# adri-romsor/iterative_inference_segm

Hardware: AMD Instinct MI355X
Metric: refined images/s (FCN-8 + standard DAE, 10-step iterative inference, 224x224, 11 classes) (higher is better)
Workload: dtype f32; 1 GPU; BASELINE configs[1]: FCN-8 + standard DAE (f64c1p2, pool4, trackind, skip), 224x224x3, batch 64/GPU, 10 steps, step 0.1, early stop off; per batch: pred_fcn_fn, val_fn, pred_dae_fn+val_fn, refine, val_fn; global_batch=64, parallelism=dp1

## Files before the change

include/iiseg.h:

```cpp
#ifndef IISEG_H
#define IISEG_H

#include <stdint.h>

#ifdef __cplusplus
extern "C" {
#endif

typedef enum iiseg_status {
    IISEG_OK = 0,
    IISEG_ERR_NULL = -1,
    IISEG_ERR_SHAPE = -2,
    IISEG_ERR_ALIGN = -3,
    IISEG_ERR_LAUNCH = -4,
    IISEG_ERR_UNSUPPORTED = -5
} iiseg_status;

const char* iiseg_strerror(int status);
const char* iiseg_last_hip_error(void);
int iiseg_abi_version(void);
const char* iiseg_target_arch(void);

int iiseg_profile_begin(int capacity);
int iiseg_profile_count(void);
// ... 14 lines not shown
    uint32_t flags;
    int32_t Kpad, Mpad;
    int32_t out_ctot, out_c0;
    int32_t out_H, out_W, out_y0, out_x0;
    int32_t tile_y0, tile_x0;
} iiseg_conv_desc;

int iiseg_conv_ktab_entries(const iiseg_conv_desc* d);
int iiseg_conv_plan(iiseg_conv_desc* d);

int iiseg_conv_pack_f32(void* stream, const iiseg_conv_desc* d, const float* w,
                        int64_t stride_o, int64_t stride_c, float* wp, int32_t* ktab);

int iiseg_conv_f32(void* stream, const iiseg_conv_desc* d, const float* x1, const float* x2,
                   const float* pre, const float* pooled, const float* wp, const int32_t* ktab,
                   const float* bias, const float* add, float* out);

int iiseg_conv_small_supported(const iiseg_conv_desc* d);
int iiseg_conv_pool_supported(const iiseg_conv_desc* d);
int iiseg_conv_pool_f32(void* stream, const iiseg_conv_desc* d, const float* x1, const float* x2,
                        const float* pre, const float* pooled, const float* wp, const int32_t* ktab,
                        const float* bias, const float* add, float* out, float* pool_out);

int iiseg_conv_mask_supported(const iiseg_conv_desc* d);
int iiseg_conv_mask_f32(void* stream, const iiseg_conv_desc* d, const float* x1, const float* x2,
                        const float* pre, const float* pooled, const uint8_t* mask_in,
                        const float* wp, const int32_t* ktab, const float* bias, const float* add,
                        float* out, float* pool_out, uint8_t* mask_out);

int iiseg_conv_halo_seam(int on);
int64_t iiseg_conv_halo_seam_launches(void);

int iiseg_conv_bnrelu_supported(const iiseg_conv_desc* d);
int iiseg_conv_bnrelu_f32(void* stream, const iiseg_conv_desc* d, const float* x, int64_t x_bstride,
                          const float* beta, const float* gamma, const float* mean,
                          const float* inv_std, const float* wp, const int32_t* ktab,
                          const float* bias, float* out);

#define IISEG_WINO_INPUT 1u
#define IISEG_WINO_GEMM 2u
#define IISEG_WINO_OUTPUT 4u
#define IISEG_WINO_ALL 7u
#define IISEG_WINO_FUSED 8u
int iiseg_conv_wino_supported(const iiseg_conv_desc* d);
int64_t iiseg_conv_wino_weight_elems(const iiseg_conv_desc* d);
int64_t iiseg_conv_wino_workspace_elems(const iiseg_conv_desc* d);
int iiseg_conv_wino_pack_f32(void* stream, const iiseg_conv_desc* d, const float* w,
                             int64_t stride_o, int64_t stride_c, float* U);
int iiseg_conv_wino_f32(void* stream, const iiseg_conv_desc* d, const float* x1, const float* x2,
                        const float* pre, const float* pooled, const float* U, const float* bias,
                        const float* add, float* workspace, float* out, uint32_t stages);
int iiseg_conv_wino_input_wide(int on);
int iiseg_conv_wino_input_path(const iiseg_conv_desc* d, int mask_bytes);
int iiseg_conv_wino_pool_supported(const iiseg_conv_desc* d);
int iiseg_conv_wino_mask_f32(void* stream, const iiseg_conv_desc* d, const float* x1, const float* x2,
                             const float* pre, const float* pooled, const uint8_t* mask_in,
                             const float* U, const float* bias, const float* add, float* workspace,
                             float* out, float* pool_out, uint8_t* mask_out, uint32_t stages);

int iiseg_conv_wino_bf16_supported(const iiseg_conv_desc* d);
int64_t iiseg_conv_wino_bf16_weight_bytes(const iiseg_conv_desc* d);
int64_t iiseg_conv_wino_bf16_workspace_bytes(const iiseg_conv_desc* d);
int iiseg_conv_wino_bf16_pack(void* stream, const iiseg_conv_desc* d, const float* w,
                              int64_t stride_o, int64_t stride_c, void* U16);
int iiseg_conv_wino_bf16(void* stream, const iiseg_conv_desc* d, const float* x1, const float* x2,
                         const float* pre, const float* pooled, const void* U16, const float* bias,
                         const float* add, void* workspace, float* out, uint32_t stages);

int iiseg_conv_gemm_bf16_supported(const iiseg_conv_desc* d);
int64_t iiseg_conv_gemm_bf16_weight_bytes(const iiseg_conv_desc* d);
int64_t iiseg_conv_gemm_bf16_workspace_bytes(const iiseg_conv_desc* d);
int iiseg_conv_gemm_bf16_pack(void* stream, const iiseg_conv_desc* d, const float* w,
                              int64_t stride_o, int64_t stride_c, void* U16);
int iiseg_conv_gemm_bf16(void* stream, const iiseg_conv_desc* d, const float* x, const void* U16,
                         const float* bias, void* workspace, float* out);

int iiseg_conv_halo_bf16_supported(const iiseg_conv_desc* d);
int64_t iiseg_conv_halo_bf16_weight_bytes(const iiseg_conv_desc* d);
int iiseg_conv_halo_bf16_pack(void* stream, const iiseg_conv_desc* d, const float* w,
                              int64_t stride_o, int64_t stride_c, void* wp16);
int iiseg_conv_halo_bf16(void* stream, const iiseg_conv_desc* d, const float* x1, const float* x2,
                         const float* pre, const float* pooled, const void* wp16, const float* bias,
                         const float* add, float* out, float* pool_out, const uint8_t* mask_in,
                         uint8_t* mask_out);

int iiseg_conv_wino_f64_supported(const iiseg_conv_desc* d);
int64_t iiseg_conv_wino_f64_weight_elems(const iiseg_conv_desc* d);
int64_t iiseg_conv_wino_f64_workspace_elems(const iiseg_conv_desc* d);
int iiseg_conv_wino_pack_f64(void* stream, const iiseg_conv_desc* d, const double* w,
                             int64_t stride_o, int64_t stride_c, double* U);
int iiseg_conv_wino_f64(void* stream, const iiseg_conv_desc* d, const double* x1, const double* x2,
                        const double* pre, const double* pooled, const double* U, const double* bias,
                        const double* add, double* workspace, double* out);

int iiseg_conv_c8_supported(const iiseg_conv_desc* d);
int iiseg_conv_c8_is_flat(const iiseg_conv_desc* d);
int iiseg_conv_c8_tiling(const iiseg_conv_desc* d, int pool, int32_t* out4);
int iiseg_conv_c8_force_tiling(int kind, int th, int tw);
int iiseg_conv_c8(void* stream, const iiseg_conv_desc* d, const void* x1, const void* x2,
                  const uint8_t* mask_in, const void* wp16, const float* bias, const void* add,
                  int add_kind, void* out, int out_kind, void* pool_out, uint8_t* mask_out);
int iiseg_conv_c8_slice(void* stream, const iiseg_conv_desc* d, const void* x1, int32_t x1_ctot,
                        const void* x2, const uint8_t* mask_in, const void* wp16, const float* bias,
                        const void* add, int add_kind, void* out, int out_kind, void* pool_out,
                        uint8_t* mask_out);
int iiseg_unpool_c8(void* stream, const void* up, const uint8_t* mask, void* out, int BC8, int H, int W,
// ... 281 lines not shown
```

iterative_inference_segm_amd/_lib.py:

```python
import ctypes as C
import os

HERE = os.path.dirname(os.path.abspath(__file__))
LIB_PATH = os.path.join(HERE, 'libiiseg_hip.so')

ABI_VERSION = 34

CONV_RELU = 1
CONV_UNPOOL = 2
CONV_X3 = 8
CONV_TRANSPOSED2 = 4
CONV_ZINS = 16


class ConvDesc(C.Structure):
    _fields_ = [(n, C.c_int32) for n in
                ('B', 'C1', 'C2', 'H', 'W', 'Cout', 'KH', 'KW', 'pad', 'dil',
                 'oy0', 'ox0', 'OH', 'OW', 'AH', 'AW', 'ay0', 'ax0')] + \
               [('flags', C.c_uint32), ('Kpad', C.c_int32), ('Mpad', C.c_int32),
                ('out_ctot', C.c_int32), ('out_c0', C.c_int32),
                ('out_H', C.c_int32), ('out_W', C.c_int32), ('out_y0', C.c_int32),
                ('out_x0', C.c_int32), ('tile_y0', C.c_int32), ('tile_x0', C.c_int32)]


# ... 10 lines not shown
class CrfDesc(C.Structure):
    _fields_ = [(n, C.c_int32) for n in ('B', 'C', 'H', 'W', 'R')] + [('flags', C.c_uint32)] + \
               [(n, C.c_double) for n in ('sxy_g', 'w_g', 'sxy_b', 'srgb', 'w_b', 'clip')]


LOSS_CROSSENTROPY = 1
LOSS_SQUARED_ERROR = 2
OPT_RMSPROP = 0
OPT_ADAM = 1


class WgradDesc(C.Structure):
    _fields_ = [(n, C.c_int32) for n in ('B', 'Cin', 'Cout', 'H', 'W', 'K', 'dil', 'gz_H', 'gz_W', 'gz_y0',
                                         'gz_x0', 'reserved')] + [('so', C.c_int64), ('sc', C.c_int64)]


class DgradDesc(C.Structure):
    _fields_ = [(n, C.c_int32) for n in ('B', 'Cin', 'Cout', 'K', 'dil', 'OH', 'OW', 'out_H', 'out_W', 'out_y0',
                                         'out_x0', 'wy0', 'wx0', 'WH', 'WW', 'ci0', 'nci', 'gx_C', 'gx_H', 'gx_W',
                                         'gx_c0', 'gx_y0', 'gx_x0', 'reserved')] + [('so', C.c_int64), ('sc', C.c_int64)]


_vp, _i32, _i64, _f32, _f64 = C.c_void_p, C.c_int32, C.c_int64, C.c_float, C.c_double

SIGNATURES = {
    'iiseg_strerror': (C.c_char_p, [C.c_int]),
    'iiseg_last_hip_error': (C.c_char_p, []),
    'iiseg_abi_version': (C.c_int, []),
    'iiseg_profile_begin': (C.c_int, [C.c_int]),
    'iiseg_profile_count': (C.c_int, []),
    'iiseg_profile_end': (C.c_int, [C.POINTER(C.c_float), C.c_int]),
    'iiseg_target_arch': (C.c_char_p, []),
    'iiseg_conv_ktab_entries': (C.c_int, [C.POINTER(ConvDesc)]),
    'iiseg_conv_plan': (C.c_int, [C.POINTER(ConvDesc)]),
    'iiseg_conv_pack_f32': (C.c_int, [_vp, C.POINTER(ConvDesc), _vp, _i64, _i64, _vp, _vp]),
    'iiseg_conv_f32': (C.c_int, [_vp, C.POINTER(ConvDesc)] + [_vp] * 9),
    'iiseg_conv_small_supported': (C.c_int, [C.POINTER(ConvDesc)]),
    'iiseg_conv_pool_supported': (C.c_int, [C.POINTER(ConvDesc)]),
    'iiseg_conv_pool_f32': (C.c_int, [_vp, C.POINTER(ConvDesc)] + [_vp] * 10),
    'iiseg_conv_halo_seam': (C.c_int, [C.c_int]),
    'iiseg_conv_halo_seam_launches': (_i64, []),
    'iiseg_conv_mask_supported': (C.c_int, [C.POINTER(ConvDesc)]),
    'iiseg_conv_mask_f32': (C.c_int, [_vp, C.POINTER(ConvDesc)] + [_vp] * 12),
    'iiseg_conv_bnrelu_supported': (C.c_int, [C.POINTER(ConvDesc)]),
    'iiseg_conv_bnrelu_f32': (C.c_int, [_vp, C.POINTER(ConvDesc), _vp, _i64] + [_vp] * 8),
    'iiseg_conv_wino_supported': (C.c_int, [C.POINTER(ConvDesc)]),
    'iiseg_conv_wino_weight_elems': (_i64, [C.POINTER(ConvDesc)]),
    'iiseg_conv_wino_workspace_elems': (_i64, [C.POINTER(ConvDesc)]),
    'iiseg_conv_wino_pack_f32': (C.c_int, [_vp, C.POINTER(ConvDesc), _vp, _i64, _i64, _vp]),
    'iiseg_conv_wino_f32': (C.c_int, [_vp, C.POINTER(ConvDesc)] + [_vp] * 9 + [C.c_uint32]),
    'iiseg_conv_wino_pool_supported': (C.c_int, [C.POINTER(ConvDesc)]),
    'iiseg_conv_wino_input_wide': (C.c_int, [C.c_int]),
    'iiseg_conv_wino_input_path': (C.c_int, [C.POINTER(ConvDesc), C.c_int]),
    'iiseg_conv_wino_mask_f32': (C.c_int, [_vp, C.POINTER(ConvDesc)] + [_vp] * 12 + [C.c_uint32]),
    'iiseg_conv_wino_bf16_supported': (C.c_int, [C.POINTER(ConvDesc)]),
    'iiseg_conv_wino_bf16_weight_bytes': (_i64, [C.POINTER(ConvDesc)]),
    'iiseg_conv_wino_bf16_workspace_bytes': (_i64, [C.POINTER(ConvDesc)]),
    'iiseg_conv_wino_bf16_pack': (C.c_int, [_vp, C.POINTER(ConvDesc), _vp, _i64, _i64, _vp]),
    'iiseg_conv_wino_bf16': (C.c_int, [_vp, C.POINTER(ConvDesc)] + [_vp] * 9 + [C.c_uint32]),
    'iiseg_conv_gemm_bf16_supported': (C.c_int, [C.POINTER(ConvDesc)]),
    'iiseg_conv_gemm_bf16_weight_bytes': (_i64, [C.POINTER(ConvDesc)]),
    'iiseg_conv_gemm_bf16_workspace_bytes': (_i64, [C.POINTER(ConvDesc)]),
    'iiseg_conv_gemm_bf16_pack': (C.c_int, [_vp, C.POINTER(ConvDesc), _vp, _i64, _i64, _vp]),
    'iiseg_conv_gemm_bf16': (C.c_int, [_vp, C.POINTER(ConvDesc)] + [_vp] * 5),
    'iiseg_conv_halo_bf16_supported': (C.c_int, [C.POINTER(ConvDesc)]),
    'iiseg_conv_halo_bf16_weight_bytes': (_i64, [C.POINTER(ConvDesc)]),
    'iiseg_conv_halo_bf16_pack': (C.c_int, [_vp, C.POINTER(ConvDesc), _vp, _i64, _i64, _vp]),
    'iiseg_conv_halo_bf16': (C.c_int, [_vp, C.POINTER(ConvDesc)] + [_vp] * 11),
    'iiseg_conv_wino_f64_supported': (C.c_int, [C.POINTER(ConvDesc)]),
    'iiseg_conv_wino_f64_weight_elems': (_i64, [C.POINTER(ConvDesc)]),
    'iiseg_conv_wino_f64_workspace_elems': (_i64, [C.POINTER(ConvDesc)]),
    'iiseg_conv_wino_pack_f64': (C.c_int, [_vp, C.POINTER(ConvDesc), _vp, _i64, _i64, _vp]),
    'iiseg_conv_wino_f64': (C.c_int, [_vp, C.POINTER(ConvDesc)] + [_vp] * 9),
    'iiseg_conv_c8_supported': (C.c_int, [C.POINTER(ConvDesc)]),
    'iiseg_conv_c8_is_flat': (C.c_int, [C.POINTER(ConvDesc)]),
    'iiseg_conv_c8_force_tiling': (C.c_int, [C.c_int, C.c_int, C.c_int]),
    'iiseg_conv_c8_tiling': (C.c_int, [C.POINTER(ConvDesc), C.c_int, C.POINTER(C.c_int32)]),
    'iiseg_conv_c8': (C.c_int, [_vp, C.POINTER(ConvDesc)] + [_vp] * 6 + [_i32, _vp, _i32, _vp, _vp]),
    'iiseg_conv_c8_slice': (C.c_int, [_vp, C.POINTER(ConvDesc), _vp, _i32] + [_vp] * 5 + [_i32, _vp, _i32, _vp, _vp]),
    'iiseg_unpool_c8': (C.c_int, [_vp] * 4 + [C.c_int] * 7),
    'iiseg_conv_c8_m16_supported': (C.c_int, [C.POINTER(ConvDesc)]),
    'iiseg_conv_c8_m16': (C.c_int, [_vp, C.POINTER(ConvDesc), _vp, _i32] + [_vp] * 6 + [_i32]),
    'iiseg_conv_c8_m16_workspace_bytes': (_i64, [C.POINTER(ConvDesc)]),
    'iiseg_conv_c8_m16_ws': (C.c_int, [_vp, C.POINTER(ConvDesc), _vp, _i32] + [_vp] * 6 + [_i32, _vp, _i64, _vp, _vp, _f64] + [_vp] * 4 + [_i32]),
    'iiseg_conv1x1_c8_weight_bytes': (_i64, [C.c_int, C.c_int]),
    'iiseg_conv1x1_c8_pack': (C.c_int, [_vp, _vp, _i64, _i64, C.c_int, C.c_int, C.c_int, _vp]),
    'iiseg_conv1x1_c8': (C.c_int, [_vp, _vp] + [C.c_int] * 5 + [_vp] * 4 + [C.c_int, C.c_int, _vp, C.c_int, C.c_int]),
    'iiseg_bn_fold_f32': (C.c_int, [_vp] * 7 + [_i32]),
    'iiseg_bn_stats_c8_workspace_elems': (C.c_int64, [_i32]),
    'iiseg_bn_stats_c8': (C.c_int, [_vp, _vp] + [_i32] * 6 + [C.c_double, _vp, _vp, _vp]),
    'iiseg_nchw_to_c8_slice': (C.c_int, [_vp, _vp, _vp] + [_i32] * 6),
    'iiseg_c8_slice_to_nchw': (C.c_int, [_vp, _vp, _vp] + [_i32] * 6),
    'iiseg_nchw_to_c8': (C.c_int, [_vp, _vp, _vp] + [_i32] * 5),
    'iiseg_c8_to_nchw': (C.c_int, [_vp, _vp, _vp] + [_i32] * 5),
    'iiseg_pool_mask_c8': (C.c_int, [_vp, _vp, _i32, _vp, _vp] + [_i32] * 11),
    'iiseg_conv_c8_split_weights': (C.c_int, [_vp, _vp, _i64, _i64, _i32, _i32, _vp]),
    'iiseg_nchw_to_c8x3': (C.c_int, [_vp, _vp, _vp] + [_i32] * 5),
    'iiseg_c8x3_to_nchw': (C.c_int, [_vp, _vp, _vp] + [_i32] * 5),
    'iiseg_pool_mask_c8x3': (C.c_int, [_vp, _vp, _vp, _vp] + [_i32] * 12),
    'iiseg_conv_gemm_supported': (C.c_int, [C.POINTER(ConvDesc)]),
    'iiseg_conv_gemm_workspace_elems': (_i64, [C.POINTER(ConvDesc)]),
    'iiseg_conv_gemm_f32': (C.c_int, [_vp, C.POINTER(ConvDesc)] + [_vp] * 5 + [C.c_uint32]),
    'iiseg_maxpool2x2_f32': (C.c_int, [_vp, _vp, _vp, _i32, _i32, _i32]),
    'iiseg_unpool_eqmask_f32': (C.c_int, [_vp, _vp, _vp, _vp, _vp, _i32, _i32, _i32]),
    'iiseg_maxpool2x2_window_f32': (C.c_int, [_vp] * 3 + [_i32] * 7),
    'iiseg_maxpool2x2_window_f64': (C.c_int, [_vp] * 3 + [_i32] * 7),
# ... 113 lines not shown
```

iterative_inference_segm_amd/csrc/conv_wino.hip:

```cpp
#include <hip/hip_runtime.h>
#include <stdint.h>
#include <stdlib.h>
#include <atomic>
#include <type_traits>
#include "iiseg.h"
#include "common.h"
#include "conv_common.h"

using namespace iiseg;

namespace {

struct WinoParams {
    const float* x1;
    const float* x2;
    const float* pre;
    const float* pooled;
    const uint8_t* mask_in;
    int h2, w2;
    const float* U;
    const float* bias;
    const float* add;
    float* V;
    float* M;
    float* out;
    int B, C1, C2, H, W;
    int Cout, pad;
    int oy0, ox0, OH, OW;
    int ty0, tx0, nty, ntx;
    int T, Tpad;
    int Kc, Mpad;
    int AH, AW, ay0, ax0;
    int relu;
    int out_ctot, out_c0, out_H, out_W, out_y0, out_x0;
    int n_ttiles, n_mtiles;
    float* pool;
    uint8_t* mask_out;
    int pool_H, pool_W;
};

__device__ __forceinline__ float pool4(float v00, float v01, float v10, float v11) {
    const float a = v00 > v01 ? v00 : v01;
    const float b = v10 > v11 ? v10 : v11;
    return a > b ? a : b;
}

__device__ __forceinline__ void pool_store(const WinoParams& p, int b, int co, int ay, int ax,
                                           float v00, float v01, float v10, float v11) {
    const float m = pool4(v00, v01, v10, v11);
    const size_t po = ((size_t)b * p.Cout + co) * p.pool_H * p.pool_W + (size_t)(ay >> 1) * p.pool_W + (ax >> 1);
    p.pool[po] = m;
    if (p.mask_out)
        p.mask_out[po] = (uint8_t)((v00 == m ? 1u : 0u) | (v01 == m ? 2u : 0u) |
                                   (v10 == m ? 4u : 0u) | (v11 == m ? 8u : 0u));
}

constexpr int RSRC_W3 = 0x00027000;

__device__ __forceinline__ __amdgpu_buffer_rsrc_t mk_rsrc(const float* base, int bytes) {
    return __builtin_amdgcn_make_buffer_rsrc((void*)base, 0, bytes, RSRC_W3);
}

__global__ void wino_weight_kernel(const float* __restrict__ w, int64_t so, int64_t sc,
                                   float* __restrict__ U, int Cin, int Cout, int Kc, int Mpad) {
    const int64_t n = (int64_t)Kc * Mpad;
    for (int64_t i = blockIdx.x * (int64_t)blockDim.x + threadIdx.x; i < n;
         i += (int64_t)gridDim.x * blockDim.x) {
        const int c = (int)(i / Mpad), co = (int)(i % Mpad);
        double g[3][3], t[4][3];
        const bool real = c < Cin && co < Cout;
#pragma unroll
        for (int a = 0; a < 3; ++a)
#pragma unroll
            for (int b = 0; b < 3; ++b) g[a][b] = real ? (double)w[co * so + c * sc + a * 3 + b] : 0.0;
#pragma unroll
        for (int b = 0; b < 3; ++b) {
            t[0][b] = g[0][b];
            t[1][b] = 0.5 * (g[0][b] + g[1][b] + g[2][b]);
            t[2][b] = 0.5 * (g[0][b] - g[1][b] + g[2][b]);
            t[3][b] = g[2][b];
        }
#pragma unroll
        for (int a = 0; a < 4; ++a) {
            const double u0 = t[a][0], u1 = 0.5 * (t[a][0] + t[a][1] + t[a][2]),
                         u2 = 0.5 * (t[a][0] - t[a][1] + t[a][2]), u3 = t[a][2];
            U[(int64_t)(a * 4 + 0) * n + i] = (float)u0;
            U[(int64_t)(a * 4 + 1) * n + i] = (float)u1;
            U[(int64_t)(a * 4 + 2) * n + i] = (float)u2;
            U[(int64_t)(a * 4 + 3) * n + i] = (float)u3;
        }
    }
}

constexpr int ICH = 4;
template <bool UNPOOL, int PY, int PX, bool MB = false>
__global__ __launch_bounds__(256) void wino_input_kernel(const WinoParams p) {
    const int t = blockIdx.x * 256 + threadIdx.x;
    if (t >= p.T) return;
    const int ntt = p.nty * p.ntx;
    const int b = t / ntt;
    const int r = t - b * ntt;
    const int tyl = r / p.ntx, txl = r - tyl * p.ntx;
    const int iy0 = p.ty0 + 2 * tyl - p.pad, ix0 = p.tx0 + 2 * txl - p.pad;
    int rowoff[4];
    bool rok[4], cok[4];
#pragma unroll
    for (int i = 0; i < 4; ++i) {
        rok[i] = (unsigned)(iy0 + i) < (unsigned)p.H;
        cok[i] = (unsigned)(ix0 + i) < (unsigned)p.W;
// ... 309 lines not shown
                v[i] = *reinterpret_cast<const float*>(src + 4u * ((pk[i] >> IW_PBITS) * ist + (pk[i] & PM)));
        }
    };

    auto run = [&](auto FULLC) __attribute__((always_inline)) {
    constexpr bool FULL = decltype(FULLC)::value;
    fetch(c0);
    for (int cc = 0; cc < chw; ++cc) {
        const int c = c0 + cc;
        float* L = Ls[cc & 1];
#pragma unroll
        for (int i = 0; i < IW_E; ++i) {
            bool on = (okm >> i) & 1u;
            if constexpr (MB) on = on && ((mq[i] >> (pk[i] & 3u)) & 1u);
            L[i * NT + tid] = on ? v[i] : 0.f;
        }
        if (cc + 1 < chw) fetch(c + 1);
        __syncthreads();
        if constexpr (!FULL)
            if (nv <= 0) continue;
        float* vo = p.V + (size_t)c * p.Tpad + q4;
#pragma unroll
        for (int i = 0; i < 4; ++i) {
            constexpr int RA[4] = {0, 1, 2, 1}, RB[4] = {2, 2, 1, 3};
            float o[4][4];
#pragma unroll
            for (int j = 0; j < 4; ++j) {
                const float* La = L + lbase[j] + RA[i] * NC;
                const float* Lb = L + lbase[j] + RB[i] * NC;
                const float2 alo = *reinterpret_cast<const float2*>(La);
                const float2 ahi = *reinterpret_cast<const float2*>(La + 2);
                const float2 blo = *reinterpret_cast<const float2*>(Lb);
                const float2 bhi = *reinterpret_cast<const float2*>(Lb + 2);
                const float da[4] = {alo.x, alo.y, ahi.x, ahi.y}, db[4] = {blo.x, blo.y, bhi.x, bhi.y};
                float e[4];
#pragma unroll
                for (int jj = 0; jj < 4; ++jj) e[jj] = i == 1 ? da[jj] + db[jj] : da[jj] - db[jj];
                o[0][j] = e[0] - e[2];
                o[1][j] = e[1] + e[2];
                o[2][j] = e[2] - e[1];
                o[3][j] = e[1] - e[3];
            }
            if (FULL || nv == 4) {
#pragma unroll
                for (int x = 0; x < 4; ++x)
                    *reinterpret_cast<float4*>(vo + (size_t)(i * 4 + x) * xis) =
                        make_float4(o[x][0], o[x][1], o[x][2], o[x][3]);
            } else {
#pragma unroll
                for (int x = 0; x < 4; ++x)
#pragma unroll
                    for (int j = 0; j < 3; ++j)
                        if (j < nv) vo[(size_t)(i * 4 + x) * xis + j] = o[x][j];
            }
        }
    }
    };
    if (tw0 + 4 * NT <= p.T) run(std::true_type{});
    else run(std::false_type{});
}

template <int BM, int BN, int WM, int WN, int NBUF, int BK = 16>
__global__ __launch_bounds__(WM * WN * 64, 2) void wino_gemm_kernel(const WinoParams p) {
    constexpr int NCH = BK / 2;
    constexpr int WTM = BM / WM, WTN = BN / WN;
    constexpr int TM = WTM / 32, TN = WTN / 32;
    constexpr int NW = WM * WN, NT = NW * 64;
    constexpr int AV = BK * BM / 4, BV = BK * BN / 4;
    constexpr int NA = NW == 8 ? 256 : NT;
    constexpr int APT = AV / NA, BPT = BV / 256;
    static_assert((NW == 4 || NW == 8) && AV % NA == 0 && BV % 256 == 0, "tile config");

    __shared__ __attribute__((aligned(16))) float As[NBUF][BK][BM];
    __shared__ __attribute__((aligned(16))) float Bs[NBUF][BK][BN];

    const int per_xi = p.n_ttiles * p.n_mtiles;
    int xi, tt, mt;
    {
        const int nb = gridDim.x, bid = blockIdx.x;
        const int q = nb / 8, r = nb % 8, xcd = bid % 8, l = bid / 8;
        const int v = (xcd < r ? xcd * (q + 1) : r * (q + 1) + (xcd - r) * q) + l;
        xi = v / per_xi;
        const int w = v - xi * per_xi;
        constexpr int GP = 8;
        const int gsize = GP * p.n_mtiles;
        const int g = w / gsize, rr = w % gsize;
        const int gp = min(GP, p.n_ttiles - g * GP);
        tt = g * GP + rr % gp;
        mt = rr / gp;
    }
    const int m0 = mt * BM, t0 = tt * BN;
    const int tid = threadIdx.x, lane = tid & 63, wave = tid >> 6;
    const int wm = wave / WN, wn = wave % WN;
    const int l31 = lane & 31, lh = lane >> 5;

    const __amdgpu_buffer_rsrc_t arsrc = mk_rsrc(p.U + (size_t)xi * p.Kc * p.Mpad, p.Kc * p.Mpad * 4);
    const __amdgpu_buffer_rsrc_t brsrc = mk_rsrc(p.V + (size_t)xi * p.Kc * p.Tpad, p.Kc * p.Tpad * 4);
    const bool bstager = NW == 4 || wave < 4;
    const bool astager = NW == 4 || wave >= 4;
    const int atid = NW == 8 ? tid - 256 : tid;
    const int awave = NW == 8 ? wave - 4 : wave;

#define WINO_STAGE(KT, BUF)                                                                        \
    {                                                                                              \
        if (astager)                                                                               \
            static_for<0, APT>([&](auto J) __attribute__((always_inline)) {                        \
// ... 380 lines not shown
                if (o && okr[i] && okc[j]) o[(ptrdiff_t)i * p.out_W + j] = v;
            }
        }
        if (p.pool && okr[1] && okc[1])
            pool_store(p, b, co, p.oy0 + wy, p.ox0 + wx, vt[0][0], vt[0][1], vt[1][0], vt[1][1]);
    }
}

inline int round_up(int v, int m) { return (v + m - 1) / m * m; }

struct WinoGeom {
    int Kc, Mpad, bm, ty0, tx0, nty, ntx, T, Tpad;
};

int wino_geom(const iiseg_conv_desc* d, WinoGeom& g) {
    if (!d) return IISEG_ERR_NULL;
    if (d->KH != 3 || d->KW != 3 || d->dil != 1 || (d->flags & IISEG_CONV_TRANSPOSED2))
        return IISEG_ERR_UNSUPPORTED;
    if ((d->flags & IISEG_CONV_UNPOOL) && d->C2 != 0) return IISEG_ERR_UNSUPPORTED;
    if (d->B <= 0 || d->C1 <= 0 || d->C2 < 0 || d->H <= 0 || d->W <= 0 || d->Cout <= 0 ||
        d->pad < 0 || d->OH <= 0 || d->OW <= 0 || d->oy0 < 0 || d->ox0 < 0)
        return IISEG_ERR_SHAPE;
    const int fullH = d->H + 2 * d->pad - 2, fullW = d->W + 2 * d->pad - 2;
    if (d->oy0 + d->OH > fullH || d->ox0 + d->OW > fullW) return IISEG_ERR_SHAPE;
    if ((d->C1 + d->C2) % 16) return IISEG_ERR_UNSUPPORTED;
    g.Kc = d->C1 + d->C2;
    g.bm = d->Cout > 128 ? 256 : (d->Cout > 64 ? 128 : 64);
    g.Mpad = round_up(d->Cout, g.bm);
    if ((d->tile_y0 | d->tile_x0) & ~1) return IISEG_ERR_SHAPE;
    g.ty0 = d->oy0 - ((d->oy0 - d->tile_y0) & 1);
    g.tx0 = d->ox0 - ((d->ox0 - d->tile_x0) & 1);
    g.nty = (d->oy0 + d->OH - g.ty0 + 1) >> 1;
    g.ntx = (d->ox0 + d->OW - g.tx0 + 1) >> 1;
    const int64_t T = (int64_t)d->B * g.nty * g.ntx;
    const int64_t Tpad = (T + 127) / 128 * 128;
    if (Tpad * g.Kc * 4 >= (int64_t)1 << 31 || (int64_t)g.Kc * g.Mpad * 4 >= (int64_t)1 << 31)
        return IISEG_ERR_UNSUPPORTED;
    g.T = (int)T;
    g.Tpad = (int)Tpad;
    return IISEG_OK;
}

std::atomic<int> g_input_wide{-1};

int input_wide_setting() {
    int v = g_input_wide.load();
    if (v < 0) {
        v = getenv("IISEG_WINO_INPUT_WIDE") ? (atoi(getenv("IISEG_WINO_INPUT_WIDE")) != 0) : 1;
        g_input_wide.store(v);
    }
    return v;
}

bool iw_fits(const WinoParams& p, int nt) {
    const int NC = 2 * p.ntx + 2;
    for (int t0 = 0; t0 < p.T; t0 += 4 * nt) {
        const int t1 = t0 + 4 * nt < p.T ? t0 + 4 * nt : p.T;
        if ((int64_t)iw_chunk(t0, t1, p.ntx, p.nty).NR * NC > (int64_t)IW_E * nt) return false;
    }
    return true;
}

int ilds_nt(const WinoParams& p);
constexpr int IW_NT = 256;

int iw_shape(const WinoParams& p, bool unpool, bool mb) {
    const int setting = input_wide_setting();
    if (!setting || (unpool && !mb)) return 0;
    if (setting != 2) {
        if (p.T < 4096) return 0;
        const int lnt = mb ? 0 : ilds_nt(p);
        if (lnt && (p.nty * p.ntx) % lnt == 0) return 0;
    }
    const int64_t HW = (int64_t)p.H * p.W, cmax = p.C1 > p.C2 ? p.C1 : p.C2;
    if (HW > (1 << IW_PBITS) || (int64_t)p.B * cmax * HW >= (int64_t)1 << 30) return 0;
    const int64_t waves1 = ((int64_t)p.T + 255) / 256 * p.Kc;
    int ch = 8;
    if (p.Kc % 32 == 0 && waves1 / 32 >= 2048) ch = 32;
    else if (waves1 / 16 >= 2048) ch = 16;
    return iw_fits(p, IW_NT) ? ch : 0;
}

int ilds_nt(const WinoParams& p) {
    static const int lds = getenv("IISEG_WINO_INPUT_LDS") ? atoi(getenv("IISEG_WINO_INPUT_LDS")) : 1;
    const int ntt = p.nty * p.ntx;
    int nt = 0;
    double best = 0.0;
    for (int cand = 256; cand >= 128; cand >>= 1) {
        const int span = (cand - 1 + p.ntx - 1) / p.ntx + 1;
        const int rows = span < p.nty ? span : p.nty;
        if ((2 * rows + 2) * (2 * p.ntx + 2) > ILDS_E * cand) continue;
        const double util = (double)ntt / (((ntt + cand - 1) / cand) * cand);
        if (util > best + 0.02) { best = util; nt = cand; }
    }
    return lds && nt && best >= 0.8 && p.Kc % ILDS_CH == 0 ? nt : 0;
}

void launch_wino_input(hipStream_t s, const WinoParams& p, bool unpool) {
    const bool mb = unpool && p.mask_in;
    if (const int chw = iw_shape(p, unpool, mb)) {
        const dim3 g2((p.T + 4 * IW_NT - 1) / (4 * IW_NT), p.Kc / chw);
        if (mb) IISEG_LAUNCH((wino_input_wide_kernel<true, IW_NT>), g2, dim3(IW_NT), 0, s, p, chw);
        else IISEG_LAUNCH((wino_input_wide_kernel<false, IW_NT>), g2, dim3(IW_NT), 0, s, p, chw);
        return;
    }
    const int nt = ilds_nt(p);
    const int ntt = p.nty * p.ntx;
    if (nt) {
        const int chunks = (ntt + nt - 1) / nt;
        const dim3 g2(p.B * chunks, p.Kc / ILDS_CH);
#define WINO_ILDS(U, N, ...) IISEG_LAUNCH((wino_input_lds_kernel<U, N, ##__VA_ARGS__>), g2, dim3(N), 0, s, p, chunks)
        if (mb) { if (nt == 256) WINO_ILDS(true, 256, true); else if (nt == 128) WINO_ILDS(true, 128, true); else WINO_ILDS(true, 64, true); }
        else if (unpool) { if (nt == 256) WINO_ILDS(true, 256); else if (nt == 128) WINO_ILDS(true, 128); else WINO_ILDS(true, 64); }
        else { if (nt == 256) WINO_ILDS(false, 256); else if (nt == 128) WINO_ILDS(false, 128); else WINO_ILDS(false, 64); }
#undef WINO_ILDS
        return;
    }
    const int nc = unpool ? ICH / 2 : ICH;
    const dim3 grid((p.T + 255) / 256, (p.Kc + nc - 1) / nc), block(256);
    if (!unpool) {
        IISEG_LAUNCH((wino_input_kernel<false, 0, 0>), grid, block, 0, s, p);
        return;
    }
    const int py = (p.ty0 - p.pad) & 1, px = (p.tx0 - p.pad) & 1;
    if (mb) {
        if (py && px) IISEG_LAUNCH((wino_input_kernel<true, 1, 1, true>), grid, block, 0, s, p);
        else if (py) IISEG_LAUNCH((wino_input_kernel<true, 1, 0, true>), grid, block, 0, s, p);
        else if (px) IISEG_LAUNCH((wino_input_kernel<true, 0, 1, true>), grid, block, 0, s, p);
        else IISEG_LAUNCH((wino_input_kernel<true, 0, 0, true>), grid, block, 0, s, p);
        return;
    }
    if (py && px) IISEG_LAUNCH((wino_input_kernel<true, 1, 1>), grid, block, 0, s, p);
    else if (py) IISEG_LAUNCH((wino_input_kernel<true, 1, 0>), grid, block, 0, s, p);
    else if (px) IISEG_LAUNCH((wino_input_kernel<true, 0, 1>), grid, block, 0, s, p);
    else IISEG_LAUNCH((wino_input_kernel<true, 0, 0>), grid, block, 0, s, p);
}

}

int iiseg_wino_output_launch(hipStream_t s, const iiseg_conv_desc* d, const float* M, int Mpad,
                             int Tpad, const float* bias, const float* add, float* out) {
    WinoParams p = {};
    p.M = const_cast<float*>(M);
    p.bias = bias; p.add = add; p.out = out;
    p.B = d->B; p.Cout = d->Cout; p.pad = d->pad;
    p.oy0 = d->oy0; p.ox0 = d->ox0; p.OH = d->OH; p.OW = d->OW;
    p.ty0 = d->oy0 - ((d->oy0 - d->tile_y0) & 1);
    p.tx0 = d->ox0 - ((d->ox0 - d->tile_x0) & 1);
    p.nty = (d->oy0 + d->OH - p.ty0 + 1) >> 1;
    p.ntx = (d->ox0 + d->OW - p.tx0 + 1) >> 1;
    p.T = d->B * p.nty * p.ntx;
    p.Tpad = Tpad; p.Mpad = Mpad;
    p.AH = d->AH; p.AW = d->AW; p.ay0 = d->ay0; p.ax0 = d->ax0;
    p.relu = (d->flags & IISEG_CONV_RELU) ? 1 : 0;
    p.out_ctot = d->out_ctot > 0 ? d->out_ctot : d->Cout;
    p.out_c0 = d->out_ctot > 0 ? d->out_c0 : 0;
    p.out_H = d->out_H > 0 ? d->out_H : d->OH;
    p.out_W = d->out_H > 0 ? d->out_W : d->OW;
    p.out_y0 = d->out_H > 0 ? d->out_y0 : 0;
    p.out_x0 = d->out_H > 0 ? d->out_x0 : 0;
    IISEG_LAUNCH(wino_output_kernel, dim3((p.T + 255) / 256, (d->Cout + OCH - 1) / OCH),
                       dim3(256), 0, s, p);
    return iiseg_check_launch();
}

extern "C" int iiseg_conv_wino_supported(const iiseg_conv_desc* d) {
    WinoGeom g;
    return wino_geom(d, g) == IISEG_OK ? 1 : 0;
}

extern "C" int iiseg_conv_wino_input_wide(int on) {
    if (on >= 0) g_input_wide.store(on > 1 ? 2 : on);
    return input_wide_setting();
}

extern "C" int iiseg_conv_wino_input_path(const iiseg_conv_desc* d, int mask_bytes) {
    WinoGeom g;
    const int st = wino_geom(d, g);
    if (st) return st;
    WinoParams p = {};
    const bool unpool = (d->flags & IISEG_CONV_UNPOOL) != 0;
    if (mask_bytes && !unpool) return IISEG_ERR_UNSUPPORTED;
    p.B = d->B; p.C1 = d->C1; p.C2 = d->C2; p.H = d->H; p.W = d->W;
    p.nty = g.nty; p.ntx = g.ntx; p.T = g.T; p.Tpad = g.Tpad; p.Kc = g.Kc;
    if (iw_shape(p, unpool, mask_bytes != 0)) return 2;
    return ilds_nt(p) ? 1 : 0;
}

extern "C" int64_t iiseg_conv_wino_weight_elems(const iiseg_conv_desc* d) {
    WinoGeom g;
    if (wino_geom(d, g) != IISEG_OK) return 0;
    return (int64_t)16 * g.Kc * g.Mpad;
}

extern "C" int64_t iiseg_conv_wino_workspace_elems(const iiseg_conv_desc* d) {
    WinoGeom g;
    if (wino_geom(d, g) != IISEG_OK) return 0;
    return (int64_t)16 * g.Tpad * ((int64_t)g.Kc + g.Mpad);
}

extern "C" int iiseg_conv_wino_pack_f32(void* stream, const iiseg_conv_desc* d, const float* w,
                                        int64_t stride_o, int64_t stride_c, float* U) {
    WinoGeom g;
    const int st = wino_geom(d, g);
    if (st) return st;
    if (!w || !U) return IISEG_ERR_NULL;
    const int64_t n = (int64_t)g.Kc * g.Mpad;
    const int grid = (int)((n + 255) / 256 < 4096 ? (n + 255) / 256 : 4096);
    IISEG_LAUNCH(wino_weight_kernel, dim3(grid), dim3(256), 0, (hipStream_t)stream, w,
                       stride_o, stride_c, U, d->C1 + d->C2, d->Cout, g.Kc, g.Mpad);
    return iiseg_check_launch();
}

static bool wino_pool_ok(const iiseg_conv_desc* d) {
    WinoGeom g;
    if (wino_geom(d, g) != IISEG_OK) return false;
    const int fullH = d->H + 2 * d->pad - 2, fullW = d->W + 2 * d->pad - 2;
    if ((d->tile_y0 | d->tile_x0 | d->oy0 | d->ox0) & 1) return false;
    if ((d->OH & 1) && d->oy0 + d->OH != fullH) return false;
    if ((d->OW & 1) && d->ox0 + d->OW != fullW) return false;
    return true;
}

extern "C" int iiseg_conv_wino_pool_supported(const iiseg_conv_desc* d) {
    return wino_pool_ok(d) ? 1 : 0;
}
// ... 288 lines not shown
```

iterative_inference_segm_amd/ops.py:

```python
import collections
import ctypes as C
import os

import torch

from . import _lib
from ._lib import ConvDesc, DeconvDesc, CONV_RELU, CONV_UNPOOL, CONV_TRANSPOSED2, CONV_X3, CONV_ZINS, check

CONV_PROFILE = None
CONV_PROFILE_INFO = None
KERNEL_BYTES = {}

_SUFFIX = {torch.float32: 'f32', torch.float64: 'f64'}

WINO_MIN_CIN = int(os.environ.get('IISEG_WINO_MIN_CIN', '128'))
WINO_F64 = os.environ.get('IISEG_WINO_F64', '1') != '0'
WINO_F64_MIN_CIN = int(os.environ.get('IISEG_WINO_F64_MIN_CIN', '128'))
WINO_F64_MIN_COUT = int(os.environ.get('IISEG_WINO_F64_MIN_COUT', '128'))
WINO_MIN_COUT = int(os.environ.get('IISEG_WINO_MIN_COUT', '128'))
WINO_FUSED_MAX_CIN = int(os.environ.get('IISEG_WINO_FUSED_MAX_CIN', '256'))
POOL_FUSE = os.environ.get('IISEG_POOL_FUSE', '1') != '0'
WINO_POOL_FUSE = os.environ.get('IISEG_WINO_POOL_FUSE', '1') != '0'
F64_POOL_FUSE = os.environ.get('IISEG_F64_POOL_FUSE', '1') != '0'
F64_MASKS = os.environ.get('IISEG_F64_MASKS', '1') != '0'
BNRELU_FUSE = os.environ.get('IISEG_BNRELU_FUSE', '0') != '0'
CONV_GEMM = os.environ.get('IISEG_CONV_GEMM', '1') != '0'
DEFAULT_MMA = os.environ.get('IISEG_MMA', 'f32')
BF16_WINO_MIN_CIN = int(os.environ.get('IISEG_BF16_WINO_MIN_CIN', '256'))
BF16_TUNE = os.environ.get('IISEG_BF16_TUNE', '0') == '1'
BF16_FORCE = os.environ.get('IISEG_BF16_FORM', '')
BF16_PICKS_FILE = os.path.join(os.path.dirname(os.path.abspath(__file__)), 'bf16_picks.json')


def _bf16_key(Cin, Cout, C1, C2, unpool, OH, OW):
    return '%d,%d,%d,%d,%d,%d,%d' % (Cin, Cout, C1, C2, 1 if unpool else 0, OH, OW)


def _load_bf16_picks():
    import json
    try:
        with open(BF16_PICKS_FILE) as f:
            return {k: v for k, v in json.load(f).get('picks', {}).items() if v in ('wino', 'halo')}
    except OSError:
        return {}


BF16_PICKS = _load_bf16_picks()
BF16_TIMES = {}


def _bf16_static_pick(Cin, OW):
    fill = OW / (32.0 * ((OW + 31) // 32))
    return 'wino' if (Cin >= 1024 or fill < 0.7) else 'halo'


C8_M16 = os.environ.get('IISEG_C8_M16', '1') != '0'
BF16_UPCONV1 = os.environ.get('IISEG_BF16_UPCONV1', '0') != '0'
BF16_WINO_MIN_COUT = int(os.environ.get('IISEG_BF16_WINO_MIN_COUT', '256'))
_SCRATCH_KINDS = {'f32': torch.float32, 'f64': torch.float64, 'bn': torch.float64, 'm16': torch.uint8}
_scratch = {}
_ws_tag = [0]


def halo_seam(on=None):
    return bool(_lib.load().iiseg_conv_halo_seam(-1 if on is None else int(bool(on))))


def halo_seam_launches():
    return int(_lib.load().iiseg_conv_halo_seam_launches())


def wino_input_wide(on=None, force=False):
    return bool(_lib.load().iiseg_conv_wino_input_wide(-1 if on is None else (2 if on and force else int(bool(on)))))


class workspace_tag:

    def __init__(self, tag):
        self.tag, self.prev = tag, None

    def __enter__(self):
        self.prev, _ws_tag[0] = _ws_tag[0], self.tag
        return self

    def __exit__(self, *exc):
        _ws_tag[0] = self.prev
        return False


def current_workspace_tag():
    return _ws_tag[0]


def _workspace(kind, n, device):
    key = (kind, device, _ws_tag[0])
    ws = _scratch.get(key)
    if ws is None or ws.numel() < n:
        _scratch[key] = None
        ws = _scratch[key] = torch.empty(int(n), dtype=_SCRATCH_KINDS[kind], device=device)
    return ws


def drop_workspaces(tag):
    for key in [k for k in _scratch if k[2] == tag]:
        _scratch.pop(key, None)


def workspace_refs(device):
    return tuple(_scratch.get((kind, device, _ws_tag[0])) for kind in _SCRATCH_KINDS)


def workspace_ptrs(device):
    return tuple(None if t is None else t.data_ptr() for t in workspace_refs(device))


_DISPATCH_TIMING = [False]
PROFILE_MS = []


class _LaunchMark:
    def __init__(self, n):
        self.n = n

    def elapsed_time(self, other):
        return float(sum(PROFILE_MS[self.n:other.n]))

# ... 1520 lines not shown
```

Baseline: 526.5 images/s.

## Stage Winograd input tiles into LDS via buffer_load...lds with double buffering

Adds a Winograd input-transform kernel that loads each channel's input patch directly from global memory into LDS using buffer_load_dword with the lds modifier. LDS is double-buffered so the next channel's loads overlap the current channel's transform. Transformed tiles are written with 128-bit buffer stores. It is enabled by default for non-mask wide-path convolutions whose input fits a 31-bit byte offset. The cost is inline asm that manipulates m0 and hand-set waitcnt values, which could be wrong on some shapes.

```diff
diff --git a/include/iiseg.h b/include/iiseg.h
--- a/include/iiseg.h
+++ b/include/iiseg.h
@@ -90,6 +90,8 @@
                         const float* add, float* workspace, float* out, uint32_t stages);
 int iiseg_conv_wino_input_wide(int on);
 int iiseg_conv_wino_input_path(const iiseg_conv_desc* d, int mask_bytes);
+int iiseg_conv_wino_input_dma(int on);
+int iiseg_conv_wino_input_staging(const iiseg_conv_desc* d, int mask_bytes);
 int iiseg_conv_wino_pool_supported(const iiseg_conv_desc* d);
 int iiseg_conv_wino_mask_f32(void* stream, const iiseg_conv_desc* d, const float* x1, const float* x2,
                              const float* pre, const float* pooled, const uint8_t* mask_in,
diff --git a/iterative_inference_segm_amd/_lib.py b/iterative_inference_segm_amd/_lib.py
--- a/iterative_inference_segm_amd/_lib.py
+++ b/iterative_inference_segm_amd/_lib.py
@@ -86,6 +86,8 @@
     'iiseg_conv_wino_pool_supported': (C.c_int, [C.POINTER(ConvDesc)]),
     'iiseg_conv_wino_input_wide': (C.c_int, [C.c_int]),
     'iiseg_conv_wino_input_path': (C.c_int, [C.POINTER(ConvDesc), C.c_int]),
+    'iiseg_conv_wino_input_dma': (C.c_int, [C.c_int]),
+    'iiseg_conv_wino_input_staging': (C.c_int, [C.POINTER(ConvDesc), C.c_int]),
     'iiseg_conv_wino_mask_f32': (C.c_int, [_vp, C.POINTER(ConvDesc)] + [_vp] * 12 + [C.c_uint32]),
     'iiseg_conv_wino_bf16_supported': (C.c_int, [C.POINTER(ConvDesc)]),
     'iiseg_conv_wino_bf16_weight_bytes': (_i64, [C.POINTER(ConvDesc)]),
diff --git a/iterative_inference_segm_amd/csrc/conv_wino.hip b/iterative_inference_segm_amd/csrc/conv_wino.hip
--- a/iterative_inference_segm_amd/csrc/conv_wino.hip
+++ b/iterative_inference_segm_amd/csrc/conv_wino.hip
@@ -55,6 +55,7 @@
                                    (v10 == m ? 4u : 0u) | (v11 == m ? 8u : 0u));
 }
 
+typedef unsigned u32x4 __attribute__((ext_vector_type(4)));
 constexpr int RSRC_W3 = 0x00027000;
 
 __device__ __forceinline__ __amdgpu_buffer_rsrc_t mk_rsrc(const float* base, int bytes) {
@@ -470,6 +471,138 @@
 #pragma unroll
                     for (int j = 0; j < 3; ++j)
                         if (j < nv) vo[(size_t)(i * 4 + x) * xis + j] = o[x][j];
+            }
+        }
+    }
+    };
+    if (tw0 + 4 * NT <= p.T) run(std::true_type{});
+    else run(std::false_type{});
+}
+
+constexpr unsigned IW_OOB = 0x80000000u;
+
+__device__ __forceinline__ void iw_dma4(i32x4s rsrc, unsigned lds, unsigned voff) {
+    unsigned keep;
+    asm volatile("s_mov_b32 %0, m0\n\ts_mov_b32 m0, %1\n\ts_nop 0\n\t"
+                 "buffer_load_dword %2, %3, 0 offen lds\n\ts_mov_b32 m0, %0"
+                 : "=&s"(keep)
+                 : "s"(lds), "v"(voff), "s"(rsrc)
+                 : "memory");
+}
+
+template <int NT>
+__global__ __launch_bounds__(NT, 3) void wino_input_dma_kernel(const WinoParams p, const int chw) {
+    __shared__ __attribute__((aligned(16))) float Ls[2][IW_E * NT];
+    const int tid = threadIdx.x;
+    const int tw0 = blockIdx.x * (4 * NT), tw1 = min(tw0 + 4 * NT, p.T);
+    const IwChunk k = iw_chunk(tw0, tw1, p.ntx, p.nty);
+    const int NC = 2 * p.ntx + 2, NE = k.NR * NC;
+    const int iyb = p.ty0 - p.pad, ixb = p.tx0 - p.pad;
+    const int HW = p.H * p.W;
+    const int c0 = blockIdx.y * chw;
+    const unsigned ist1 = (unsigned)(p.C1 * HW), ist2 = (unsigned)(p.C2 * HW);
+    unsigned voff[IW_E];
+    {
+        const unsigned ist = c0 < p.C1 ? ist1 : ist2;
+#pragma unroll
+        for (int i = 0; i < IW_E; ++i) {
+            const int e = i * NT + tid;
+            const int r = e / NC, c = e - r * NC;
+            int bi = 0, ry = 2 * k.tyf + r;
+            if (r >= k.R0) {
+                const int r2 = r - k.R0;
+                bi = r2 / k.RI;
+                ry = r2 - bi * k.RI;
+                bi += 1;
+            }
+            const int iy = iyb + ry, ix = ixb + c;
+            const bool ok = e < NE && (unsigned)iy < (unsigned)p.H && (unsigned)ix < (unsigned)p.W;
+            voff[i] = ok ? 4u * ((unsigned)bi * ist + (unsigned)(iy * p.W + ix)) : IW_OOB;
+        }
+    }
+    const int q4 = tw0 + 4 * tid;
+    int lbase[4];
+#pragma unroll
+    for (int j = 0; j < 4; ++j) {
+        const int t = min(q4 + j, tw1 - 1);
+        const int gr = t / p.ntx, txl = t - gr * p.ntx;
+        const int b = gr / p.nty, ty = gr - b * p.nty;
+        const int row = b == k.b0 ? 2 * (ty - k.tyf) : k.R0 + (b - k.b0 - 1) * k.RI + 2 * ty;
+        lbase[j] = row * NC + 2 * txl;
+    }
+    const int nv = min(4, tw1 - q4);
+    const size_t xis = (size_t)p.Kc * p.Tpad;
+    const int vbytes = p.Kc * p.Tpad * 4;
+    const unsigned lds0 = lds_addr(&Ls[0][0]) + 256u * (unsigned)__builtin_amdgcn_readfirstlane(tid >> 6);
+
+    auto stage = [&](int c, int buf) __attribute__((always_inline)) {
+        const bool first = c < p.C1;
+        const int cs = first ? p.C1 : p.C2, cl = first ? c : c - p.C1;
+        const float* base = (first ? p.x1 : p.x2) + ((size_t)k.b0 * cs + cl) * HW;
+        const i32x4s rs = mk_srsrc(base, 4u * (unsigned)(((p.B - k.b0) * cs - cl) * HW));
+        const unsigned l = lds0 + (unsigned)buf * (unsigned)(IW_E * NT * 4);
+#pragma unroll
+        for (int i = 0; i < IW_E; ++i) iw_dma4(rs, l + (unsigned)(i * NT * 4), voff[i]);
+    };
+
+    stage(c0, 0);
+    auto run = [&](auto FULLC) __attribute__((always_inline)) {
+    constexpr bool FULL = decltype(FULLC)::value;
+    for (int cc = 0; cc < chw; ++cc) {
+        const int c = c0 + cc;
+        bool fresh = cc == 0;
+        if (cc > 0 && c == p.C1) {
+#pragma unroll
+            for (int i = 0; i < IW_E; ++i)
+                if (voff[i] != IW_OOB) voff[i] += 4u * (ist2 - ist1) * (voff[i] / (4u * ist1));
+            stage(c, cc & 1);
+            fresh = true;
+        }
+        if (FULL && !fresh) asm volatile("s_waitcnt vmcnt(16) lgkmcnt(0)" ::: "memory");
+        else asm volatile("s_waitcnt vmcnt(0) lgkmcnt(0)" ::: "memory");
+        __builtin_amdgcn_s_barrier();
+        asm volatile("" ::: "memory");
+        if (cc + 1 < chw && c + 1 != p.C1) stage(c + 1, (cc + 1) & 1);
+        if constexpr (!FULL)
+            if (nv <= 0) continue;
+        const float* L = Ls[cc & 1];
+        const int vo = 4 * (c * p.Tpad + q4);
+#pragma unroll
+        for (int i = 0; i < 4; ++i) {
+            constexpr int RA[4] = {0, 1, 2, 1}, RB[4] = {2, 2, 1, 3};
+            float o[4][4];
+#pragma unroll
+            for (int j = 0; j < 4; ++j) {
+                const float* La = L + lbase[j] + RA[i] * NC;
+                const float* Lb = L + lbase[j] + RB[i] * NC;
+                const float2 alo = *reinterpret_cast<const float2*>(La);
+                const float2 ahi = *reinterpret_cast<const float2*>(La + 2);
+                const float2 blo = *reinterpret_cast<const float2*>(Lb);
+                const float2 bhi = *reinterpret_cast<const float2*>(Lb + 2);
+                const float da[4] = {alo.x, alo.y, ahi.x, ahi.y}, db[4] = {blo.x, blo.y, bhi.x, bhi.y};
+                float e[4];
+#pragma unroll
+                for (int jj = 0; jj < 4; ++jj) e[jj] = i == 1 ? da[jj] + db[jj] : da[jj] - db[jj];
+                o[0][j] = e[0] - e[2];
+                o[1][j] = e[1] + e[2];
+                o[2][j] = e[2] - e[1];
+                o[3][j] = e[1] - e[3];
+            }
+            if (FULL || nv == 4) {
+#pragma unroll
+                for (int x = 0; x < 4; ++x)
+                    __builtin_amdgcn_raw_buffer_store_b128(
+                        __builtin_bit_cast(u32x4, make_float4(o[x][0], o[x][1], o[x][2], o[x][3])),
+                        mk_rsrc(p.V + (size_t)(i * 4 + x) * xis, vbytes), vo, 0, 0);
+            } else {
+#pragma unroll
+                for (int x = 0; x < 4; ++x)
+#pragma unroll
+                    for (int j = 0; j < 3; ++j)
+                        if (j < nv)
+                            __builtin_amdgcn_raw_buffer_store_b32(
+                                __builtin_bit_cast(unsigned, o[x][j]),
+                                mk_rsrc(p.V + (size_t)(i * 4 + x) * xis, vbytes), vo + 4 * j, 0, 0);
             }
         }
     }
@@ -956,6 +1089,17 @@
     return v;
 }
 
+std::atomic<int> g_input_dma{-1};
+
+int input_dma_setting() {
+    int v = g_input_dma.load();
+    if (v < 0) {
+        v = getenv("IISEG_WINO_INPUT_DMA") ? (atoi(getenv("IISEG_WINO_INPUT_DMA")) != 0) : 1;
+        g_input_dma.store(v);
+    }
+    return v;
+}
+
 bool iw_fits(const WinoParams& p, int nt) {
     const int NC = 2 * p.ntx + 2;
     for (int t0 = 0; t0 < p.T; t0 += 4 * nt) {
@@ -983,6 +1127,12 @@
     if (p.Kc % 32 == 0 && waves1 / 32 >= 2048) ch = 32;
     else if (waves1 / 16 >= 2048) ch = 16;
     return iw_fits(p, IW_NT) ? ch : 0;
+}
+
+int iw_staging(const WinoParams& p, bool mb) {
+    if (mb || !input_dma_setting()) return 1;
+    const int64_t HW = (int64_t)p.H * p.W, cmax = p.C1 > p.C2 ? p.C1 : p.C2;
+    return (int64_t)p.B * cmax * HW * 4 < (int64_t)1 << 31 ? 2 : 1;
 }
 
 int ilds_nt(const WinoParams& p) {
@@ -1004,7 +1154,8 @@
     const bool mb = unpool && p.mask_in;
     if (const int chw = iw_shape(p, unpool, mb)) {
         const dim3 g2((p.T + 4 * IW_NT - 1) / (4 * IW_NT), p.Kc / chw);
-        if (mb) IISEG_LAUNCH((wino_input_wide_kernel<true, IW_NT>), g2, dim3(IW_NT), 0, s, p, chw);
+        if (iw_staging(p, mb) == 2) IISEG_LAUNCH((wino_input_dma_kernel<IW_NT>), g2, dim3(IW_NT), 0, s, p, chw);
+        else if (mb) IISEG_LAUNCH((wino_input_wide_kernel<true, IW_NT>), g2, dim3(IW_NT), 0, s, p, chw);
         else IISEG_LAUNCH((wino_input_wide_kernel<false, IW_NT>), g2, dim3(IW_NT), 0, s, p, chw);
         return;
     }
@@ -1076,6 +1227,23 @@
 extern "C" int iiseg_conv_wino_input_wide(int on) {
     if (on >= 0) g_input_wide.store(on > 1 ? 2 : on);
     return input_wide_setting();
+}
+
+extern "C" int iiseg_conv_wino_input_dma(int on) {
+    if (on >= 0) g_input_dma.store(on ? 1 : 0);
+    return input_dma_setting();
+}
+
+extern "C" int iiseg_conv_wino_input_staging(const iiseg_conv_desc* d, int mask_bytes) {
+    WinoGeom g;
+    const int st = wino_geom(d, g);
+    if (st) return st;
+    WinoParams p = {};
+    const bool unpool = (d->flags & IISEG_CONV_UNPOOL) != 0;
+    if (mask_bytes && !unpool) return IISEG_ERR_UNSUPPORTED;
+    p.B = d->B; p.C1 = d->C1; p.C2 = d->C2; p.H = d->H; p.W = d->W;
+    p.nty = g.nty; p.ntx = g.ntx; p.T = g.T; p.Tpad = g.Tpad; p.Kc = g.Kc;
+    return iw_shape(p, unpool, mask_bytes != 0) ? iw_staging(p, mask_bytes != 0) : 0;
 }
 
 extern "C" int iiseg_conv_wino_input_path(const iiseg_conv_desc* d, int mask_bytes) {
diff --git a/iterative_inference_segm_amd/ops.py b/iterative_inference_segm_amd/ops.py
--- a/iterative_inference_segm_amd/ops.py
+++ b/iterative_inference_segm_amd/ops.py
@@ -72,6 +72,10 @@
 
 def wino_input_wide(on=None, force=False):
     return bool(_lib.load().iiseg_conv_wino_input_wide(-1 if on is None else (2 if on and force else int(bool(on)))))
+
+
+def wino_input_dma(on=None):
+    return bool(_lib.load().iiseg_conv_wino_input_dma(-1 if on is None else int(bool(on))))
 
 
 class workspace_tag:
```

Measured after the change: 526.9 images/s, median of 4. Within noise of the previous version (+0.1%).
